# cszheng-ioa/Sixty-years-of-frequency-domain-monaural-speech-enhancement

Hardware: AMD Instinct MI355X
Metric: utterances/sec, 16 kHz 4 s clips, DCCRN decode (STFT->network->iSTFT) (higher is better)
Workload: dtype f32; 1 GPU; BASELINE configs[2]: DCCRN complex-mask, compressed input (0.5/2.0), 16 kHz x 4 s clips, batch 256 per MI355X, utterance-sharded; batch_per_gpu=256, global_batch=256, clip_samples=64000, parallelism=utterance shard x1 + RCCL gather to rank 0

## Files before the change

### sixty-years-of-frequency-domain-monaural-speech-enhancement_amd/csrc/engine.hip

```cpp
#include "../../include/se_engine.h"
#include "hip_owned.h"
#include "model.h"
#include "resampler.h"
#include "rnn.h"
#include "stream_manifest.h"
#include "k_stream_state.h"
#include "stream_join.h"
#include "stream_rows.h"
#include "stream_window.h"
#include "window_rows.h"
#include <cmath>
#include <algorithm>
#include <climits>
#include <cstring>
#include <mutex>

using namespace se;

struct se_engine {
    se_config cfg{};
    EngineCtx ctx;
    StateDict sd;
    std::unique_ptr<Model> model;
    bool finalized = false;
    int plan_frames = 0;
    std::string err;
    struct GraphEntry {
        int batch, samples;
        hipGraphExec_t exec;
    };
    std::vector<GraphEntry> graphs;
    std::vector<std::pair<int, int>> warmed;
    DevBuf<float> stage_in, stage_out;
    DevBuf<float> hook_buf;
    size_t hook_cap = 0;
    static constexpr int RAG_SLOTS = 8;
    PinnedBuf<int> rag_host;
    DevBuf<int> rag_dev;
    Event rag_ev[RAG_SLOTS];
    int rag_next = 0;
    DevBuf<int> rag_win;
    OwnedStream cap_stream;
    Event ev_fork, ev_join;
    static constexpr int MAX_TWINS = 2;
    int ntwins = 0;
    std::unique_ptr<EngineCtx> ctx2[MAX_TWINS];
    std::unique_ptr<Model> twin[MAX_TWINS];
    Event ev_tfork, ev_tjoin[MAX_TWINS];
    struct Stream {
        bool active = false;
        int batch = 0, max_chunk = 0, n_total = 0, t_done = 0, o_done = 0;
        int w0 = 0;
        long pitch = 0;
        DevBuf<float> wav, wav2;
        const float* ext = nullptr;
        long ext_pitch = 0;
        int carve_B = -1, carve_n = -1;
        bool running = false;
        DevBuf<double> sumsq;
        DevBuf<float> frame_inv;
        int ring = 0;
        DevBuf<float> c;
        bool tracking = false;
        float tau = 0.f;
        double lam = 1.0;
        DevBuf<float> frame_c;
        bool per_frame() const { return running || tracking; }
        int scale_mode() const { return tracking ? 2 : running ? 1 : 0; }
        bool has_last = false;
        hipStream_t last_st = nullptr;
        Event ev_order;
        void start(int batch_, int n_total_, bool running_, bool tracking_ = false, float tau_ = 0.f, int hop = 1) {
            batch = batch_;
            n_total = n_total_;
            running = running_;
            tracking = tracking_;
            tau = tracking_ ? tau_ : 0.f;
            lam = tracking_ && tau_ > 0.f ? std::exp(-(double)hop / (double)tau_) : 1.0;
            t_done = o_done = w0 = 0;
            carve_B = carve_n = -1;
            ext = nullptr;
        }
    } strm;
};

static std::string g_create_err;

template <typename F>
static int guard(se_engine* e, F&& f) {
    int prev = -1;
    int rc = 0;
    try {
        if (e) {
            SE_HIP(hipGetDevice(&prev));
            if (prev != e->cfg.device) SE_HIP(hipSetDevice(e->cfg.device));
            else prev = -1;
        }
        f();
    } catch (const std::exception& ex) {
        if (e) e->err = ex.what();
        else g_create_err = ex.what();
        rc = 1;
    }
    if (prev >= 0) (void)hipSetDevice(prev);
    return rc;
}

struct StageProfScope {
    explicit StageProfScope(se_engine* e) { set_stage_prof(e->ctx.prof.on ? &e->ctx.stage_prof : nullptr); }
    ~StageProfScope() { set_stage_prof(nullptr); }
};

extern "C" {

int64_t se_resample_samples(int32_t n_in, int32_t sr_in, int32_t sr_out) {
    if (n_in <= 0 || sr_in <= 0 || sr_out <= 0) return -1;
    return se::resample_out_samples(n_in, sr_in, sr_out);
}

int se_resample(const float* in_dev, int64_t in_pitch, int32_t batch, int32_t n_in, int32_t sr_in, int32_t sr_out,
                float* out_dev, int64_t out_pitch, void* stream) {
    return guard(nullptr, [&] {
        SE_CHECK(in_dev && out_dev, "null argument");
        SE_CHECK(in_pitch >= n_in && out_pitch >= se::resample_out_samples(n_in, sr_in, sr_out), "row pitch too small");
        se::launch_resample(in_dev, in_pitch, batch, n_in, sr_in, sr_out, out_dev, out_pitch, static_cast<hipStream_t>(stream));
    });
}

int se_resample_ragged(const void* in_dev, int32_t in_format, int64_t in_pitch, int32_t batch, const int32_t* n_in, int32_t sr_in,
                       int32_t sr_out, float* out_dev, int64_t out_pitch, void* stream) {
    return guard(nullptr, [&] {
        se::launch_resample_ragged(in_dev, in_format, in_pitch, batch, n_in, sr_in, sr_out, out_dev, out_pitch, static_cast<hipStream_t>(stream));
    });
}

static se::StreamResampler* rs_of(se_resampler* r) { return reinterpret_cast<se::StreamResampler*>(r); }

int se_resampler_create(int32_t sr_in, int32_t sr_out, int32_t max_batch, int32_t max_push, se_resampler** out) {
    return guard(nullptr, [&] {
        SE_CHECK(out, "null argument");
        *out = reinterpret_cast<se_resampler*>(se::stream_resampler_create(sr_in, sr_out, max_batch, max_push));
    });
}
int se_resampler_destroy(se_resampler* r) {
    return guard(nullptr, [&] { se::stream_resampler_destroy(rs_of(r)); });
}
int se_resampler_begin(se_resampler* r, int32_t batch, void* stream) {
    return guard(nullptr, [&] {
        SE_CHECK(r, "null argument");
        se::stream_resampler_begin(rs_of(r), batch, static_cast<hipStream_t>(stream));
    });
}
int se_resampler_push(se_resampler* r, const float* in_dev, int64_t in_pitch, int32_t n_new, float* out_dev, int64_t out_pitch,
                      int32_t* n_out, void* stream) {
    return guard(nullptr, [&] {
        SE_CHECK(r && n_out, "null argument");
        *n_out = se::stream_resampler_push(rs_of(r), in_dev, in_pitch, n_new, out_dev, out_pitch, static_cast<hipStream_t>(stream));
    });
}
int se_resampler_flush(se_resampler* r, float* out_dev, int64_t out_pitch, int32_t* n_out, void* stream) {
    return guard(nullptr, [&] {
        SE_CHECK(r && n_out, "null argument");
        *n_out = se::stream_resampler_flush(rs_of(r), out_dev, out_pitch, static_cast<hipStream_t>(stream));
    });
}
int64_t se_resampler_ready_samples(int64_t n_in, int32_t sr_in, int32_t sr_out) {
    return se::resample_ready_samples(n_in, sr_in, sr_out);
}

static se::ResamplerState* rst_of(const se_resampler_state* s) {
    return reinterpret_cast<se::ResamplerState*>(const_cast<se_resampler_state*>(s));
}

int se_resampler_state_create(se_resampler_state** out) {
    return guard(nullptr, [&] {
        SE_CHECK(out, "se_resampler_state_create: null argument");
        *out = reinterpret_cast<se_resampler_state*>(se::resampler_state_create());
    });
}
int se_resampler_state_destroy(se_resampler_state* s) {
    return guard(nullptr, [&] { se::resampler_state_destroy(rst_of(s)); });
}
int64_t se_resampler_state_bytes(const se_resampler_state* s) { return se::resampler_state_bytes(rst_of(s)); }
int se_resampler_state_counts(const se_resampler_state* s, int32_t* sr_in, int32_t* sr_out, int32_t* batch, int64_t* n_in, int64_t* n_out) {
    return guard(nullptr, [&] { se::resampler_state_counts(rst_of(s), sr_in, sr_out, batch, n_in, n_out); });
}
int se_resampler_save(se_resampler* r, se_resampler_state* s, void* stream) {
    return guard(nullptr, [&] {
        SE_CHECK(r && s, "se_resampler_save: null argument");
        se::stream_resampler_save(rs_of(r), rst_of(s), static_cast<hipStream_t>(stream));
    });
}
int se_resampler_restore(se_resampler* r, const se_resampler_state* s, void* stream) {
    return guard(nullptr, [&] {
        SE_CHECK(r && s, "se_resampler_restore: null argument");
        se::stream_resampler_restore(rs_of(r), rst_of(s), static_cast<hipStream_t>(stream));
    });
}
int64_t se_resampler_state_export(const se_resampler_state* s, void* host_buf, int64_t cap) {
    int64_t ret = -1;
    guard(nullptr, [&] { ret = se::resampler_state_export(rst_of(s), host_buf, cap); });
    return ret;
}
int se_resampler_state_import(se_resampler_state* s, const void* host_buf, int64_t bytes) {
    return guard(nullptr, [&] { se::resampler_state_import(rst_of(s), host_buf, bytes); });
}

int se_resampler_state_select(se_resampler_state* dst, const se_resampler_state* src, const int32_t* rows, int32_t n_rows, void* stream) {
    return guard(nullptr, [&] { se::resampler_state_select(rst_of(dst), rst_of(src), rows, n_rows, static_cast<hipStream_t>(stream)); });
}
int se_resampler_state_concat(se_resampler_state* dst, const se_resampler_state* const* parts, int32_t n_parts, void* stream) {
    return guard(nullptr, [&] {
        se::resampler_state_concat(rst_of(dst), reinterpret_cast<se::ResamplerState* const*>(const_cast<se_resampler_state* const*>(parts)), n_parts,
                                   static_cast<hipStream_t>(stream));
    });
}
int se_resampler_state_join(se_resampler_state* dst, const se_resampler_state* const* parts, int32_t n_parts, void* stream) {
    return guard(nullptr, [&] {
        se::resampler_state_join(rst_of(dst), reinterpret_cast<se::ResamplerState* const*>(const_cast<se_resampler_state* const*>(parts)), n_parts,
                                 static_cast<hipStream_t>(stream));
    });
}

int se_pcm16_decode(const int16_t* in_dev, int64_t in_pitch, int32_t batch, int32_t n, float* out_dev, int64_t out_pitch,
                    void* stream) {
    return guard(nullptr, [&] {
        SE_CHECK(in_dev && out_dev, "null argument");
        SE_CHECK(batch == 1 || (in_pitch >= n && out_pitch >= n), "row pitch too small");
        se::launch_pcm16_decode(in_dev, in_pitch, batch, n, out_dev, out_pitch, static_cast<hipStream_t>(stream));
    });
}

int se_pcm16_encode(const float* in_dev, int64_t in_pitch, int32_t batch, int32_t n, int16_t* out_dev, int64_t out_pitch,
                    void* stream) {
    return guard(nullptr, [&] {
        SE_CHECK(in_dev && out_dev, "null argument");
        SE_CHECK(batch == 1 || (in_pitch >= n && out_pitch >= n), "row pitch too small");
        se::launch_pcm16_encode(in_dev, in_pitch, batch, n, out_dev, out_pitch, static_cast<hipStream_t>(stream));
    });
}

int32_t se_abi_version(void) { return 5; }

const char* se_last_error(const se_engine* e) { return e ? e->err.c_str() : g_create_err.c_str(); }

static std::unique_ptr<Model> make_model(int id, EngineCtx& c) {
    switch (id) {
        case SE_MODEL_DCCRN: return make_dccrn(c);
        case SE_MODEL_CRN: return make_crn(c);
        case SE_MODEL_LSTM: return make_lstm(c);
        case SE_MODEL_DPCRN: return make_dpcrn(c);
        case SE_MODEL_GCRN: return make_gcrn(c);
        case SE_MODEL_CTSNET: return make_ctsnet(c);
        case SE_MODEL_TAYLORSENET: return make_taylorsenet(c);
        case SE_MODEL_G2NET: return make_g2net(c);
        case SE_MODEL_UFORMER: return make_uformer(c);
        case SE_MODEL_FULLSUBNET: return make_fullsubnet(c);
        default: SE_CHECK(false, "model id " + std::to_string(id) + " is not built into this engine yet");
    }
    return nullptr;
}
static hipStream_t twin_stream(int dev, int i = 0) { return EngineCtx::shared_aux(dev, i); }

int se_engine_create(const se_config* cfg, se_engine** out) {
    se_engine* e = nullptr;
    int prev_dev = -1;
    (void)hipGetDevice(&prev_dev);
    int rc = guard(nullptr, [&] {
        SE_CHECK(cfg && out, "null argument");
        int ndev = 0;
        SE_HIP(hipGetDeviceCount(&ndev));
        SE_CHECK(ndev > 0, "no HIP device visible: the engine has no CPU fallback");
        SE_CHECK(cfg->device >= 0 && cfg->device < ndev, "device ordinal out of range");
        SE_HIP(hipSetDevice(cfg->device));
        hipDeviceProp_t prop;
        SE_HIP(hipGetDeviceProperties(&prop, cfg->device));
        SE_CHECK(std::string(prop.gcnArchName).rfind("gfx950", 0) == 0,
                 std::string("built for gfx950 (MI355X) only, device is ") + prop.gcnArchName);
        e = new se_engine();
        e->cfg = *cfg;
        e->ctx.max_batch = cfg->max_batch > 0 ? cfg->max_batch : 1;
        e->ctx.max_samples = cfg->max_samples > 0 ? cfg->max_samples : 64000;
        e->ctx.p_in = cfg->p_in > 0.f ? cfg->p_in : 1.f;
        e->ctx.p_out = cfg->p_out > 0.f ? cfg->p_out : 1.f;
        e->ctx.flags = cfg->flags;
        e->model = make_model(cfg->model, e->ctx);
        e->ctx.geom = e->model->default_geom();
        if (cfg->n_fft > 0) {
            SE_CHECK(cfg->n_fft == e->ctx.geom.n_fft, "n_fft override must match the model's front end");
            e->ctx.geom = StftGeom{cfg->n_fft, cfg->hop > 0 ? cfg->hop : e->ctx.geom.hop, cfg->win > 0 ? cfg->win : cfg->n_fft};
        }
        static const int split_env = getenv("SE_BATCH_SPLIT") ? atoi(getenv("SE_BATCH_SPLIT")) : -1;
        const bool split = split_env >= 0 ? split_env != 0
                                          : (cfg->model == SE_MODEL_UFORMER || cfg->model == SE_MODEL_DPCRN || cfg->model == SE_MODEL_CTSNET ||
                                             cfg->model == SE_MODEL_TAYLORSENET);
        if (split && e->ctx.max_batch >= 64) {
            const int parts = (cfg->model == SE_MODEL_UFORMER || cfg->model == SE_MODEL_DPCRN) ? 3 : 2;
            e->ntwins = parts - 1;
            for (int i = 0; i < e->ntwins; ++i) {
                e->ctx2[i].reset(new EngineCtx());
                e->ctx2[i]->max_batch = (e->ctx.max_batch + i + 1) / (i + 2);
                e->ctx2[i]->max_samples = e->ctx.max_samples;
                e->ctx2[i]->p_in = e->ctx.p_in;
                e->ctx2[i]->p_out = e->ctx.p_out;
                e->ctx2[i]->flags = e->ctx.flags;
                e->twin[i] = make_model(cfg->model, *e->ctx2[i]);
                e->ctx2[i]->geom = e->ctx.geom;
            }
        }
        *out = e;
        scratch_engine_created(cfg->device);
    });
    if (rc && e) {
        delete e;
    }
    if (prev_dev >= 0) (void)hipSetDevice(prev_dev);
    return rc;
}

int se_engine_destroy(se_engine* e) {
    if (!e) return 0;
    int prev_dev = -1;
    (void)hipGetDevice(&prev_dev);
    (void)hipSetDevice(e->cfg.device);
    (void)hipDeviceSynchronize();
    for (auto& g : e->graphs)
        if (g.exec) (void)hipGraphExecDestroy(g.exec);
    if (e->ctx.arena.base()) gc_unregister_overread_range(e->ctx.arena.base());
    for (auto& c2 : e->ctx2)
        if (c2 && c2->arena.base()) gc_unregister_overread_range(c2->arena.base());
    const int dev = e->cfg.device;
    delete e;
    scratch_engine_destroyed(dev);
    if (prev_dev >= 0) (void)hipSetDevice(prev_dev);
    return 0;
}

int se_engine_set_tensor(se_engine* e, const char* key, const void* data, const int64_t* shape, int32_t ndim,
                         int32_t dtype) {
    if (!e) return 1;
    return guard(e, [&] {
        SE_CHECK(!e->finalized, "set_tensor after finalize");
        SE_CHECK(key && (data || ndim == 0) && ndim >= 0 && ndim <= 8, "bad argument");
        HostTensor t;
        int64_t n = 1;
        for (int i = 0; i < ndim; ++i) {
            SE_CHECK(shape[i] >= 0, "negative dim");
            t.shape.push_back(shape[i]);
            n *= shape[i];
        }
        if (dtype == 0) {
            t.data.assign(static_cast<const float*>(data), static_cast<const float*>(data) + n);
        } else if (dtype == 1) {
            t.data.resize(n);
            for (int64_t i = 0; i < n; ++i) t.data[i] = (float)static_cast<const int64_t*>(data)[i];
        } else {
            SE_CHECK(false, "dtype must be 0 (float32) or 1 (int64)");
        }
        e->sd[key] = std::move(t);
    });
}

int se_engine_finalize(se_engine* e) {
    if (!e) return 1;
    return guard(e, [&] {
        SE_CHECK(!e->finalized, "already finalized");
        TrackedSD tsd(e->sd);
        e->model->finalize(tsd);
        tsd.check_all_used();
        const int T = e->model->num_frames(e->ctx.max_samples);
        const int fm = pad_frames_mult(e->model->frame_multiple());
        const int Tr = (T + fm - 1) / fm * fm;
        e->plan_frames = e->model->stream_supported() ? std::max(Tr, e->model->stream_hc() + 16) : Tr;
        size_t need = 0;
        for (int bq : {e->ctx.max_batch, std::min(e->ctx.max_batch, 15)})
            for (int tq : {e->plan_frames, std::min(e->plan_frames, 64)}) {
                if (tq != e->plan_frames && !e->model->stream_supported()) continue;
                e->ctx.arena.measure_begin();
                e->model->plan_buffers(bq, tq);
                need = std::max(need, e->ctx.arena.measure_end());
            }
        e->ctx.arena.reserve(need + (1 << 20));
        gc_register_overread_range(e->ctx.arena.base(), e->ctx.arena.capacity());
        e->model->plan_buffers(e->ctx.max_batch, T);
        for (int i = 0; i < e->ntwins; ++i) {
            TrackedSD tsd2(e->sd);
            e->twin[i]->finalize(tsd2);
            size_t need2 = 0;
            for (int bq : {e->ctx2[i]->max_batch, std::min(e->ctx2[i]->max_batch, 15)}) {
                e->ctx2[i]->arena.measure_begin();
                e->twin[i]->plan_buffers(bq, Tr);
                need2 = std::max(need2, e->ctx2[i]->arena.measure_end());
            }
            e->ctx2[i]->arena.reserve(need2 + (1 << 20));
            gc_register_overread_range(e->ctx2[i]->arena.base(), e->ctx2[i]->arena.capacity());
            e->twin[i]->plan_buffers(e->ctx2[i]->max_batch, T);
        }
        e->sd.clear();
        SE_HIP(hipDeviceSynchronize());
        e->finalized = true;
    });
}

static void stream_mark(se_engine::Stream& S, hipStream_t st) {
    SE_HIP(hipEventRecord(S.ev_order.get(), st));
    S.has_last = true;
    S.last_st = st;
}
static void stream_order_wait(se_engine::Stream& S, hipStream_t st) {
    if (S.has_last && S.last_st != st) SE_HIP(hipStreamWaitEvent(st, S.ev_order.get(), 0));
}
struct ArenaCall {
    enum Mode { MARK_ONLY, RECARVE, TAKE_OVER };
    se_engine::Stream& S;
    hipStream_t st;
    ArenaCall(se_engine* e, hipStream_t st_, Mode mode = RECARVE) : S(e->strm), st(st_) {
        if (mode == MARK_ONLY) return;
        if (mode == TAKE_OVER) S.active = false;
        S.carve_B = -1;
        stream_order_wait(S, st);
    }
    ~ArenaCall() {
        try {
            stream_mark(S, st);
        } catch (const std::exception&) {
        }
    }
    ArenaCall(const ArenaCall&) = delete;
    ArenaCall& operator=(const ArenaCall&) = delete;
};

int se_forward(se_engine* e, const float* in_dev, const int64_t* in_shape, int32_t in_ndim, float* out_dev,
               void* stream) {
    if (!e) return 1;
    return guard(e, [&] {
        SE_CHECK(e->finalized, "engine not finalized");
        ArenaCall call(e, static_cast<hipStream_t>(stream));
        SE_CHECK(in_dev && out_dev && in_shape, "null argument");
        e->ctx.prof_reset();
        e->model->forward(in_dev, in_shape, in_ndim, out_dev, static_cast<hipStream_t>(stream));
    });
}

int se_uformer_forward(se_engine* e, const float* inputs_dev, const float* src_dev, int32_t batch, int32_t n_samples,
                       float* output_dev, float* src_out_dev, float* output_cplx_dev, float* src_cplx_dev, void* stream) {
    if (!e) return 1;
    return guard(e, [&] {
        SE_CHECK(e->finalized, "engine not finalized");
        ArenaCall call(e, static_cast<hipStream_t>(stream));
        SE_CHECK(inputs_dev && output_dev, "null argument");
        SE_CHECK(batch >= 1 && batch <= e->ctx.max_batch, "batch exceeds max_batch given at create");
        SE_CHECK(n_samples >= e->ctx.geom.n_fft && n_samples <= e->ctx.max_samples, "n_samples outside [n_fft, max_samples]");
        e->ctx.prof_reset();
        e->model->forward_uformer(inputs_dev, src_dev, batch, n_samples, output_dev, src_out_dev, output_cplx_dev, src_cplx_dev,
                                  static_cast<hipStream_t>(stream));
    });
}

int se_enhance_batch(se_engine* e, const float* wav_in_dev, int64_t in_pitch, int32_t batch, int32_t n_samples,
                     float* wav_out_dev, int64_t out_pitch, void* stream) {
    if (!e) return 1;
    return guard(e, [&] {
        SE_CHECK(e->finalized, "engine not finalized");
        ArenaCall call(e, static_cast<hipStream_t>(stream));
        SE_CHECK(wav_in_dev && wav_out_dev, "null argument");
        SE_CHECK(batch >= 1 && batch <= e->ctx.max_batch, "batch exceeds max_batch given at create");
        SE_CHECK(n_samples >= e->ctx.geom.n_fft && n_samples <= e->ctx.max_samples,
                 "n_samples outside [n_fft, max_samples]");
        SE_CHECK(in_pitch >= n_samples && out_pitch >= e->model->output_samples(n_samples), "row pitch too small");
        e->ctx.prof_reset();
        StageProfScope sps(e);
        hipStream_t st = static_cast<hipStream_t>(stream);
        static const int graphs_env = getenv("SE_GRAPH") ? atoi(getenv("SE_GRAPH")) : -1;
        const bool want_graph = (graphs_env >= 0 ? graphs_env != 0 : (e->cfg.flags & SE_CFG_GRAPHS) != 0) && !e->ctx.prof.on &&
                                e->model->graph_capturable();
        if (!want_graph) {
            if (e->ntwins > 0 && !e->ctx.prof.on && batch >= 64) {
                const int parts = (e->ntwins >= 2 && batch >= 192) ? 3 : 2;
                const int Bp = (batch + parts - 1) / parts;
                struct Active {
                    Active() { batch_split_active() = true; }
                    ~Active() { batch_split_active() = false; }
                } active;
                struct TwinJoin {
                    se_engine* e;
                    hipStream_t st;
                    int n = 0;
                    ~TwinJoin() {
                        try {
                            for (int i = 0; i < n; ++i) (void)hipStreamWaitEvent(st, e->ev_tjoin[i].get(), 0);
                        } catch (const std::exception&) {
                        }
                    }
                } join{e, st};
                SE_HIP(hipEventRecord(e->ev_tfork.get(), st));
                for (int i = 0; i < parts - 1; ++i) {
                    const int r0 = (i + 1) * Bp, nr = std::min(Bp, batch - r0);
                    if (nr <= 0) break;
                    hipStream_t s2 = twin_stream(e->cfg.device, i);
                    SE_HIP(hipStreamWaitEvent(s2, e->ev_tfork.get(), 0));
                    e->twin[i]->enhance(wav_in_dev + (size_t)r0 * in_pitch, in_pitch, nr, n_samples, wav_out_dev + (size_t)r0 * out_pitch,
                                        out_pitch, s2);
                    SE_HIP(hipEventRecord(e->ev_tjoin[i].get(), s2));
                    join.n = i + 1;
                }
                e->model->enhance(wav_in_dev, in_pitch, std::min(Bp, batch), n_samples, wav_out_dev, out_pitch, st);
                return;
            }
            e->model->enhance(wav_in_dev, in_pitch, batch, n_samples, wav_out_dev, out_pitch, st);
            return;
        }
        const int64_t n_out = e->model->output_samples(n_samples);
        se_engine::GraphEntry* ge = nullptr;
        for (auto& g : e->graphs)
            if (g.batch == batch && g.samples == n_samples) ge = &g;
        if (!ge) {
            const std::pair<int, int> key(batch, n_samples);
            hipStream_t cs = e->cap_stream.get();
            if (std::find(e->warmed.begin(), e->warmed.end(), key) == e->warmed.end()) {
                e->warmed.push_back(key);
                SE_HIP(hipEventRecord(e->ev_fork.get(), st));
                SE_HIP(hipStreamWaitEvent(cs, e->ev_fork.get(), 0));
                e->model->enhance(wav_in_dev, in_pitch, batch, n_samples, wav_out_dev, out_pitch, cs);
                SE_HIP(hipEventRecord(e->ev_join.get(), cs));
                SE_HIP(hipStreamWaitEvent(st, e->ev_join.get(), 0));
                return;
            }
            if (!e->stage_in) {
                const int64_t max_out = e->model->output_samples(e->ctx.max_samples);
                e->stage_in.alloc((size_t)e->ctx.max_batch * e->ctx.max_samples);
                e->stage_out.alloc((size_t)e->ctx.max_batch * max_out);
            }
            hipGraph_t graph = nullptr;
            hipGraphExec_t exec = nullptr;
            SE_HIP(hipStreamBeginCapture(cs, hipStreamCaptureModeThreadLocal));
            bool ok = true;
            try {
                e->model->enhance(e->stage_in.get(), n_samples, batch, n_samples, e->stage_out.get(), n_out, cs);
            } catch (const std::exception&) {
                ok = false;
            }
            if (hipStreamEndCapture(cs, &graph) != hipSuccess || !graph) ok = false;
            if (ok && hipGraphInstantiate(&exec, graph, nullptr, nullptr, 0) != hipSuccess) ok = false;
            if (graph) (void)hipGraphDestroy(graph);
            (void)hipGetLastError();
            if (getenv("SE_GRAPH_DEBUG"))
                fprintf(stderr, "se_graph: %s (batch %d, samples %d)\n", ok ? "captured" : "capture failed", batch, n_samples);
            e->graphs.push_back({batch, n_samples, ok ? exec : nullptr});
            ge = &e->graphs.back();
        }
        if (!ge->exec) {
            e->model->enhance(wav_in_dev, in_pitch, batch, n_samples, wav_out_dev, out_pitch, st);
            return;
        }
        SE_HIP(hipMemcpy2DAsync(e->stage_in.get(), (size_t)n_samples * sizeof(float), wav_in_dev, (size_t)in_pitch * sizeof(float),
                                (size_t)n_samples * sizeof(float), batch, hipMemcpyDeviceToDevice, st));
        SE_HIP(hipGraphLaunch(ge->exec, st));
        SE_HIP(hipMemcpy2DAsync(wav_out_dev, (size_t)out_pitch * sizeof(float), e->stage_out.get(), (size_t)n_out * sizeof(float),
                                (size_t)n_out * sizeof(float), batch, hipMemcpyDeviceToDevice, st));
    });
}

static Ragged upload_row_sizes(se_engine* e, int batch, const int32_t* lengths, hipStream_t st) {
    const int MB = e->ctx.max_batch;
    if (!e->rag_host) {
        e->rag_host.alloc((size_t)4 * MB * se_engine::RAG_SLOTS);
        e->rag_dev.alloc((size_t)4 * MB * se_engine::RAG_SLOTS);
    }
    const int slot = e->rag_next;
    e->rag_next = (slot + 1) % se_engine::RAG_SLOTS;
    SE_HIP(hipEventSynchronize(e->rag_ev[slot].get()));
    int* h = e->rag_host.get() + (size_t)slot * 4 * MB;
    int* d = e->rag_dev.get() + (size_t)slot * 4 * MB;
    const int hop = e->ctx.geom.hop;
    for (int b = 0; b < batch; ++b) {
        const int L = lengths[b], Lp = e->model->padded_samples(L);
        h[b] = L;
        h[MB + b] = Lp;
        h[2 * MB + b] = 1 + Lp / hop;
        h[3 * MB + b] = (int)e->model->output_samples(L);
    }
    SE_HIP(hipMemcpyAsync(d, h, sizeof(int) * 4 * MB, hipMemcpyHostToDevice, st));
    SE_HIP(hipEventRecord(e->rag_ev[slot].get(), st));
    return Ragged{d, d + MB, d + 2 * MB, d + 3 * MB};
}
struct RaggedScope {
    const bool on;
    explicit RaggedScope(const Ragged* r) : on(r != nullptr) {
        if (on) set_ragged_ctx(r);
    }
    ~RaggedScope() {
        if (on) set_ragged_ctx(nullptr);
    }
    RaggedScope(const RaggedScope&) = delete;
    RaggedScope& operator=(const RaggedScope&) = delete;
};

int se_enhance_ragged(se_engine* e, const float* wav_in_dev, int64_t in_pitch, int32_t batch, const int32_t* lengths,
                      float* wav_out_dev, int64_t out_pitch, void* stream) {
    if (!e) return 1;
    return guard(e, [&] {
        SE_CHECK(e->finalized, "engine not finalized");
        ArenaCall call(e, static_cast<hipStream_t>(stream));
        SE_CHECK(wav_in_dev && wav_out_dev && lengths, "null argument");
        SE_CHECK(batch >= 1 && batch <= e->ctx.max_batch, "batch exceeds max_batch given at create");
        SE_CHECK(e->model->ragged_supported(),
                 "this model looks ahead in time (non-causal convolutions / attention): batch only clips of equal length");
        int Lmax = 0;
        for (int b = 0; b < batch; ++b) {
            SE_CHECK(lengths[b] >= e->ctx.geom.n_fft && lengths[b] <= e->ctx.max_samples,
                     "lengths[" + std::to_string(b) + "] outside [n_fft, max_samples]");
            Lmax = std::max(Lmax, (int)lengths[b]);
        }
        SE_CHECK(in_pitch >= Lmax && out_pitch >= e->model->output_samples(Lmax), "row pitch too small");
        hipStream_t st = static_cast<hipStream_t>(stream);
        const Ragged rg = upload_row_sizes(e, batch, lengths, st);
        e->ctx.prof_reset();
        StageProfScope sps(e);
        RaggedScope scope(&rg);
        e->model->enhance(wav_in_dev, in_pitch, batch, Lmax, wav_out_dev, out_pitch, st);
    });
}

static void stream_process(se_engine* e, int t_end, bool last, float* out_dev, int64_t out_pitch, int* written, hipStream_t st,
                           const Ragged* rows = nullptr) {
    se_engine::Stream& S = e->strm;
    const float* wav = S.ext ? S.ext : S.wav.get();
    const long pitch = S.ext ? S.ext_pitch : S.pitch;
    const int w0 = S.w0;
    const StftGeom& g = e->ctx.geom;
    const int HC = e->model->stream_hc(), LAG = e->model->stream_lag(), B = S.batch;
    const int Lpad = last ? e->model->padded_samples(S.n_total) : S.n_total;
    const int n_final = last ? (int)e->model->output_samples(S.n_total) : S.n_total;
    const int MB = e->ctx.max_batch;
    if (rows && !e->rag_win) e->rag_win.alloc((size_t)4 * MB);
    int* const rw = e->rag_win.get();
    const Ragged win{rw, rw + MB, rw + 2 * MB, rw + 3 * MB};
    const Ragged* view = rows ? &win : nullptr;
    while (S.t_done < t_end) {
        const int t0 = S.t_done, n = std::min(S.max_chunk, t_end - t0), Tw = HC + n;
        float *spec = nullptr, *mag = nullptr, *est = nullptr;
        e->model->stream_bufs(B, n, &spec, &mag, &est);
        if (S.carve_B != B || S.carve_n != n) {
            SE_HIP(hipMemsetAsync(const_cast<void*>(e->ctx.arena.base()), 0, e->ctx.arena.used(), st));
            S.carve_B = B;
            S.carve_n = n;
        }
        {
            if (rows) launch_window_rows(rows->len, rw, MB, B, t0 + n, st);
            RaggedScope rs(view);
            launch_stft(g, wav, pitch, B, S.n_total, Lpad, S.c.get(), e->ctx.p_in, spec, mag, t0 + n, Tw, st, t0, HC, w0,
                        S.tracking ? S.frame_c.get() : nullptr, S.ring);
        }
        e->model->stream_chunk(B, t0, n, st, last && t0 + n == t_end);
        S.t_done = t0 + n;
        const bool end = last && S.t_done == t_end;
        const int t_fin = end ? S.t_done : S.t_done - LAG;
        const int o_hi = end ? n_final : std::min(S.n_total, t_fin * g.hop - g.n_fft / 2);
        if (o_hi > S.o_done) {
            if (rows && t_fin != t0 + n) launch_window_rows(rows->len, rw, MB, B, t_fin, st);
            RaggedScope rs(view);
            launch_istft(g, est, B, t_fin, Tw, nullptr, S.per_frame() ? nullptr : S.c.get(), out_dev + *written, out_pitch, o_hi, st, t0 - HC,
                         std::max(0, t0 - HC), S.o_done, S.per_frame() ? S.frame_inv.get() : nullptr, S.ring);
            *written += o_hi - S.o_done;
            S.o_done = o_hi;
        }
    }
}

static void check_stream_geometry(const se_engine* e) {
    const StftGeom& g = e->ctx.geom;
    SE_CHECK((g.n_fft + g.hop - 1) / g.hop - 1 + e->model->stream_lag() <= e->model->stream_hc(),
             "front end overlap + look-ahead exceed the history the model keeps");
}
static int window_frames(const se_engine* e, int requested, int dflt) {
    const int room = std::max(1, e->plan_frames - e->model->stream_hc());
    return std::min(requested > 0 ? requested : dflt, room);
}

static void scale_rings_alloc(se_engine* e, bool tracking) {
    se_engine::Stream& S = e->strm;
    if (!S.sumsq) {
        S.ring = 64;
        while (S.ring < e->plan_frames + 64) S.ring <<= 1;
        S.sumsq.alloc((size_t)2 * e->ctx.max_batch);
        S.frame_inv.alloc((size_t)e->ctx.max_batch * S.ring);
    }
    if (tracking && !S.frame_c) S.frame_c.alloc((size_t)e->ctx.max_batch * S.ring);
}

static int stream_begin_impl(se_engine* e, int32_t batch, int32_t max_chunk_frames, const float* c_dev, bool running, void* stream,
                             bool tracking = false, float tau = 0.f) {
    if (!e) return 1;
    return guard(e, [&] {
        SE_CHECK(e->finalized, "engine not finalized");
        e->strm.carve_B = -1;
        if (tracking)
            SE_CHECK(std::isfinite(tau) && tau >= 0.f,
                     "se_stream_begin_tracking: tau_samples has to be a finite number >= 0 (0: never forget), got " + std::to_string(tau));
        SE_CHECK(e->model->stream_supported(), "this model has no frame-online mode (CRN, LSTM, GCRN, DPCRN, DCCRN, FullSubNet with the cumulative norm and the cLN `_new` weights of CTSNet / TaylorSENet / G2Net have)");
        SE_CHECK(batch >= 1 && batch <= e->ctx.max_batch, "batch exceeds max_batch given at create");
        check_stream_geometry(e);
        const StftGeom& g = e->ctx.geom;
        if (tracking)
            SE_CHECK(g.n_fft >= 2 * g.hop - 2, "se_stream_begin_tracking: n_fft " + std::to_string(g.n_fft) + " < 2 hop - 2 (hop " + std::to_string(g.hop) +
                                                   "): the stream's input window does not keep the head of an incomplete hop block");
        hipStream_t st = static_cast<hipStream_t>(stream);
        se_engine::Stream& S = e->strm;
        stream_order_wait(S, st);
        S.max_chunk = window_frames(e, max_chunk_frames, 16);
        if (!S.wav) {
            const bool sliding = (e->cfg.flags & SE_CFG_STREAM_SLIDING) != 0;
            S.pitch = sliding ? stream_window_pitch(e->ctx.max_samples, g.n_fft, g.hop) : e->ctx.max_samples;
            S.wav.alloc((size_t)e->ctx.max_batch * S.pitch);
            if (sliding) S.wav2.alloc((size_t)e->ctx.max_batch * S.pitch);
        }
        if (!S.c) S.c.alloc(e->ctx.max_batch);
        if (c_dev) SE_HIP(hipMemcpyAsync(S.c.get(), c_dev, (size_t)batch * sizeof(float), hipMemcpyDeviceToDevice, st));
        else launch_fill(S.c.get(), batch, 1.f, st);
        if (running || tracking) {
            scale_rings_alloc(e, tracking);
            SE_HIP(hipMemsetAsync(S.sumsq.get(), 0, (size_t)batch * (tracking ? 2 : 1) * sizeof(double), st));
            launch_fill(S.frame_inv.get(), (long)batch * S.ring, 1.f, st);
            if (tracking) launch_fill(S.frame_c.get(), (long)batch * S.ring, 1.f, st);
        }
        S.start(batch, 0, running, tracking, tau, g.hop);
        e->model->stream_begin(batch, S.max_chunk, st);
        S.active = true;
        stream_mark(S, st);
    });
}

int se_stream_begin(se_engine* e, int32_t batch, int32_t max_chunk_frames, const float* c_dev, void* stream) {
    return stream_begin_impl(e, batch, max_chunk_frames, c_dev, false, stream);
}
int se_stream_begin_running(se_engine* e, int32_t batch, int32_t max_chunk_frames, void* stream) {
    return stream_begin_impl(e, batch, max_chunk_frames, nullptr, true, stream);
}

int se_stream_begin_tracking(se_engine* e, int32_t batch, int32_t max_chunk_frames, float tau_samples, void* stream) {
    return stream_begin_impl(e, batch, max_chunk_frames, nullptr, false, stream, true, tau_samples);
}

int se_stream_scale(se_engine* e, float* c_dev, void* stream) {
    if (!e) return 1;
    return guard(e, [&] {
        se_engine::Stream& S = e->strm;
        SE_CHECK(S.active, "se_stream_scale without se_stream_begin");
        SE_CHECK(c_dev, "se_stream_scale: null argument");
        hipStream_t st = static_cast<hipStream_t>(stream);
        stream_order_wait(S, st);
        SE_HIP(hipMemcpyAsync(c_dev, S.c.get(), (size_t)S.batch * sizeof(float), hipMemcpyDeviceToDevice, st));
        stream_mark(S, st);
    });
}

int se_stream_push(se_engine* e, const float* wav_dev, int64_t pitch, int32_t n_new, float* out_dev, int64_t out_pitch,
                   int32_t* n_out, void* stream) {
    if (!e) return 1;
    return guard(e, [&] {
        se_engine::Stream& S = e->strm;
        SE_CHECK(S.active, "se_stream_push without se_stream_begin");
        SE_CHECK(wav_dev && out_dev && n_out && n_new >= 0, "bad argument");
        SE_CHECK(S.batch == 1 || pitch >= n_new, "se_stream_push: input row pitch smaller than n_new");
        const StftGeom& g = e->ctx.geom;
        const bool sliding = (e->cfg.flags & SE_CFG_STREAM_SLIDING) != 0;
        int keep = S.w0;
        if (sliding) {
            SE_CHECK(n_new <= e->ctx.max_samples, "se_stream_push: a single push may carry at most max_samples samples");
            SE_CHECK((int64_t)S.n_total + n_new <= stream_sample_limit(e->ctx.max_samples, g.n_fft, g.hop),
                     "sliding stream longer than 2^31 - 1 - max_samples samples");
            if ((long)(S.n_total - S.w0) + n_new > S.pitch) {
                keep = stream_keep_from(g.n_fft, g.hop, S.t_done, S.n_total);
                SE_CHECK(keep >= S.w0 && keep <= S.n_total && (long)(S.n_total - keep) + n_new <= S.pitch,
                         "se_stream_push: the stream window cannot hold this push behind the samples still to be transformed");
            }
        } else {
            SE_CHECK(S.n_total + n_new <= e->ctx.max_samples, "stream longer than max_samples given at create");
        }
        hipStream_t st = static_cast<hipStream_t>(stream);
        ArenaCall call(e, st, ArenaCall::MARK_ONLY);
        if (keep != S.w0) {
            launch_stream_slide(S.wav.get(), S.wav2.get(), S.pitch, S.batch, keep - S.w0, (S.n_total - keep + 3) & ~3, st);
            std::swap(S.wav, S.wav2);
            S.w0 = keep;
        }
        if (n_new > 0)
            SE_HIP(hipMemcpy2DAsync(S.wav.get() + (S.n_total - S.w0), (size_t)S.pitch * sizeof(float), wav_dev,
                                    (size_t)pitch * sizeof(float), (size_t)n_new * sizeof(float), S.batch,
                                    hipMemcpyDeviceToDevice, st));
        S.n_total += n_new;
        const int t_avail = S.n_total > g.n_fft / 2 ? (S.n_total - g.n_fft / 2 - 1) / g.hop + 1 : 0;
        if (S.tracking)
            launch_stream_track(g, S.wav.get(), S.pitch, S.batch, S.n_total, n_new, false, S.lam, S.sumsq.get(), S.c.get(), S.frame_c.get(),
                                S.frame_inv.get(), S.ring, S.t_done, std::max(t_avail, S.t_done), st, S.w0);
        else if (S.running)
            launch_stream_rms(S.wav.get(), S.pitch, S.batch, S.n_total, n_new, S.sumsq.get(), S.c.get(), S.frame_inv.get(), S.ring, S.t_done,
                              std::max(t_avail, S.t_done), st, S.w0);
        int written = 0;
        const int will = std::max(0, std::min(S.n_total, (t_avail - e->model->stream_lag()) * g.hop - g.n_fft / 2) - S.o_done);
        SE_CHECK(out_pitch >= will, "output row pitch too small for the samples this push completes");
        e->ctx.prof_reset();
        stream_process(e, std::max(t_avail, S.t_done), false, out_dev, out_pitch, &written, st);
        *n_out = written;
    });
}

int se_stream_flush(se_engine* e, float* out_dev, int64_t out_pitch, int32_t* n_out, void* stream) {
    if (!e) return 1;
// ... 956 lines not shown
```

Measured before the change: 2618 utt/s.

## Enable concurrent batch splitting for DCCRN with configurable part count and lead

Adds DCCRN to the models whose batch is split across twin model instances running on separate streams, so a batch of 256 runs as two concurrent halves by default. Also factors the split into a helper that supports unequal leading-part sizes and env-configurable part counts. The intent is to overlap the partly serial recurrent and small-kernel work of independent sub-batches and fill the GPU better. The cost is extra workspace memory for a twin model and possible contention between the streams.

```diff
diff --git a/sixty-years-of-frequency-domain-monaural-speech-enhancement_amd/csrc/batch_parts.h b/sixty-years-of-frequency-domain-monaural-speech-enhancement_amd/csrc/batch_parts.h
--- /dev/null
+++ b/sixty-years-of-frequency-domain-monaural-speech-enhancement_amd/csrc/batch_parts.h
@@ -0,0 +1,66 @@
+#pragma once
+
+namespace se {
+
+constexpr int BATCH_PARTS_MAX = 3;
+constexpr int BATCH_SPLIT_MIN = 64;
+constexpr int BATCH_LEAD_EQUAL = 8;
+constexpr int BATCH_LEAD_MIN = 4, BATCH_LEAD_MAX = 12;
+
+struct BatchParts {
+    int n = 1;
+    int r0[BATCH_PARTS_MAX] = {};
+    int rows[BATCH_PARTS_MAX] = {};
+};
+
+inline int batch_parts_count(int batch, int ntwins) {
+    if (ntwins <= 0 || batch < BATCH_SPLIT_MIN) return 1;
+    const int have = ntwins + 1 < BATCH_PARTS_MAX ? ntwins + 1 : BATCH_PARTS_MAX;
+    return have >= 3 && batch >= 192 ? 3 : 2;
+}
+
+inline BatchParts batch_parts_cut(int batch, int parts, int lead) {
+    BatchParts p;
+    p.rows[0] = batch > 0 ? batch : 0;
+    if (parts > BATCH_PARTS_MAX) parts = BATCH_PARTS_MAX;
+    if (batch <= 0 || parts <= 1) return p;
+    if (lead == BATCH_LEAD_EQUAL) {
+        const int Bp = (int)(((long long)batch + parts - 1) / parts);
+        p.n = 0;
+        for (int i = 0; i < parts && (long long)i * Bp < batch; ++i) {
+            p.r0[i] = i * Bp;
+            p.rows[i] = batch - i * Bp < Bp ? batch - i * Bp : Bp;
+            p.n = i + 1;
+        }
+        return p;
+    }
+    if (batch < 4 * parts) return p;
+    lead = lead < BATCH_LEAD_MIN ? BATCH_LEAD_MIN : lead > BATCH_LEAD_MAX ? BATCH_LEAD_MAX : lead;
+    int r = 0;
+    for (int i = 0; i < parts; ++i) {
+        const int k = parts - i, left = batch - r;
+        int take = left;
+        if (k > 1) {
+            const long long num = (long long)left * lead, den = 8LL * k;
+            take = (int)((2 * num + 4 * den) / (8 * den)) * 4;
+            const int hi = (left - 4 * (k - 1)) & ~3;
+            take = take < 4 ? 4 : take > hi ? hi : take;
+        }
+        p.r0[i] = r;
+        p.rows[i] = take;
+        r += take;
+    }
+    p.n = parts;
+    return p;
+}
+
+inline int batch_parts_twin_rows(int max_batch, int ntwins, int lead, int twin) {
+    int m = 0;
+    for (int b = BATCH_SPLIT_MIN; b <= max_batch; ++b) {
+        const BatchParts p = batch_parts_cut(b, batch_parts_count(b, ntwins), lead);
+        if (twin + 1 < p.n && p.rows[twin + 1] > m) m = p.rows[twin + 1];
+    }
+    return m;
+}
+
+}
diff --git a/sixty-years-of-frequency-domain-monaural-speech-enhancement_amd/csrc/engine.hip b/sixty-years-of-frequency-domain-monaural-speech-enhancement_amd/csrc/engine.hip
--- a/sixty-years-of-frequency-domain-monaural-speech-enhancement_amd/csrc/engine.hip
+++ b/sixty-years-of-frequency-domain-monaural-speech-enhancement_amd/csrc/engine.hip
@@ -3,6 +3,7 @@
 #include "model.h"
 #include "resampler.h"
 #include "rnn.h"
+#include "batch_parts.h"
 #include "stream_manifest.h"
 #include "k_stream_state.h"
 #include "stream_join.h"
@@ -42,8 +43,9 @@
     DevBuf<int> rag_win;
     OwnedStream cap_stream;
     Event ev_fork, ev_join;
-    static constexpr int MAX_TWINS = 2;
+    static constexpr int MAX_TWINS = BATCH_PARTS_MAX - 1;
     int ntwins = 0;
+    int split_lead = BATCH_LEAD_EQUAL;
     std::unique_ptr<EngineCtx> ctx2[MAX_TWINS];
     std::unique_ptr<Model> twin[MAX_TWINS];
     Event ev_tfork, ev_tjoin[MAX_TWINS];
@@ -291,15 +293,20 @@
             e->ctx.geom = StftGeom{cfg->n_fft, cfg->hop > 0 ? cfg->hop : e->ctx.geom.hop, cfg->win > 0 ? cfg->win : cfg->n_fft};
         }
         static const int split_env = getenv("SE_BATCH_SPLIT") ? atoi(getenv("SE_BATCH_SPLIT")) : -1;
+        static const int parts_env = getenv("SE_BATCH_PARTS") ? atoi(getenv("SE_BATCH_PARTS")) : 0;
+        static const int lead_env = getenv("SE_BATCH_LEAD") ? atoi(getenv("SE_BATCH_LEAD")) : 0;
         const bool split = split_env >= 0 ? split_env != 0
                                           : (cfg->model == SE_MODEL_UFORMER || cfg->model == SE_MODEL_DPCRN || cfg->model == SE_MODEL_CTSNET ||
-                                             cfg->model == SE_MODEL_TAYLORSENET);
-        if (split && e->ctx.max_batch >= 64) {
-            const int parts = (cfg->model == SE_MODEL_UFORMER || cfg->model == SE_MODEL_DPCRN) ? 3 : 2;
+                                             cfg->model == SE_MODEL_TAYLORSENET || cfg->model == SE_MODEL_DCCRN);
+        if (split && e->ctx.max_batch >= BATCH_SPLIT_MIN) {
+            const int parts = parts_env >= 1 && parts_env <= BATCH_PARTS_MAX ? parts_env
+                              : (cfg->model == SE_MODEL_UFORMER || cfg->model == SE_MODEL_DPCRN) ? 3 : 2;
             e->ntwins = parts - 1;
+            e->split_lead = lead_env >= BATCH_LEAD_MIN && lead_env <= BATCH_LEAD_MAX ? lead_env : BATCH_LEAD_EQUAL;
             for (int i = 0; i < e->ntwins; ++i) {
                 e->ctx2[i].reset(new EngineCtx());
-                e->ctx2[i]->max_batch = (e->ctx.max_batch + i + 1) / (i + 2);
+                e->ctx2[i]->max_batch = e->split_lead == BATCH_LEAD_EQUAL ? (e->ctx.max_batch + i + 1) / (i + 2)
+                                                                          : std::max(1, batch_parts_twin_rows(e->ctx.max_batch, e->ntwins, e->split_lead, i));
                 e->ctx2[i]->max_samples = e->ctx.max_samples;
                 e->ctx2[i]->p_in = e->ctx.p_in;
                 e->ctx2[i]->p_out = e->ctx.p_out;
@@ -475,9 +482,8 @@
         const bool want_graph = (graphs_env >= 0 ? graphs_env != 0 : (e->cfg.flags & SE_CFG_GRAPHS) != 0) && !e->ctx.prof.on &&
                                 e->model->graph_capturable();
         if (!want_graph) {
-            if (e->ntwins > 0 && !e->ctx.prof.on && batch >= 64) {
-                const int parts = (e->ntwins >= 2 && batch >= 192) ? 3 : 2;
-                const int Bp = (batch + parts - 1) / parts;
+            const BatchParts bp = e->ctx.prof.on ? BatchParts() : batch_parts_cut(batch, batch_parts_count(batch, e->ntwins), e->split_lead);
+            if (bp.n > 1) {
                 struct Active {
                     Active() { batch_split_active() = true; }
                     ~Active() { batch_split_active() = false; }
@@ -494,9 +500,9 @@
                     }
                 } join{e, st};
                 SE_HIP(hipEventRecord(e->ev_tfork.get(), st));
-                for (int i = 0; i < parts - 1; ++i) {
-                    const int r0 = (i + 1) * Bp, nr = std::min(Bp, batch - r0);
-                    if (nr <= 0) break;
+                for (int i = 0; i < bp.n - 1; ++i) {
+                    const int r0 = bp.r0[i + 1], nr = bp.rows[i + 1];
+                    SE_CHECK(nr <= e->ctx2[i]->max_batch, "a part of the batch exceeds its instance's workspace");
                     hipStream_t s2 = twin_stream(e->cfg.device, i);
                     SE_HIP(hipStreamWaitEvent(s2, e->ev_tfork.get(), 0));
                     e->twin[i]->enhance(wav_in_dev + (size_t)r0 * in_pitch, in_pitch, nr, n_samples, wav_out_dev + (size_t)r0 * out_pitch,
@@ -504,7 +510,7 @@
                     SE_HIP(hipEventRecord(e->ev_tjoin[i].get(), s2));
                     join.n = i + 1;
                 }
-                e->model->enhance(wav_in_dev, in_pitch, std::min(Bp, batch), n_samples, wav_out_dev, out_pitch, st);
+                e->model->enhance(wav_in_dev, in_pitch, bp.rows[0], n_samples, wav_out_dev, out_pitch, st);
                 return;
             }
             e->model->enhance(wav_in_dev, in_pitch, batch, n_samples, wav_out_dev, out_pitch, st);
```

Result: faster. 2648 utt/s, median of 6 (+1.1%).
